# zakuro-ai/asr

Hardware: AMD Instinct MI355X
Metric: utterances/sec (10 s, 161-bin) DS2 5x1024 BiGRU CTC train step (higher is better)
Workload: dtype bf16

## Files before the change

asr_amd/_lib.py:

```python
from __future__ import annotations

import ctypes as C
import os
from typing import Optional

_HERE = os.path.dirname(os.path.abspath(__file__))
LIB_PATH = os.environ.get("DS2_LIB_PATH") or os.path.join(_HERE, "lib", "libds2hip.so")

_lib: Optional[C.CDLL] = None

vp, i32, i64, f32, f64, sz = C.c_void_p, C.c_int, C.c_longlong, C.c_float, C.c_double, C.c_size_t

SIGNATURES = {
    "ds2_version": (C.c_char_p, []),
    "ds2_last_error": (C.c_char_p, []),
    "ds2_device_info": (i32, [C.POINTER(i32), C.POINTER(i32), C.c_char_p, i32]),
    "ds2_debug_flags": (i32, [vp, i32]),
    "ds2_rnn_ctx_init": (i32, [vp, vp, vp, vp]),
    "ds2_memset_async": (i32, [vp, i32, sz, vp]),
    "ds2_ablation_build": (i32, []),
    "ds2_rnn_persistent_status": (i32, [vp, vp]),
    "ds2_rnn_persistent_counters": (i32, [vp, vp]),
    "ds2_rnn_poison_if_starved": (i32, [vp, vp, sz, vp]),
    "ds2_rnn_poison_seen": (i32, [vp]),
# ... 55 lines not shown
    "ds2_conv_wgrad_workspace_bytes": (sz, [i32, i32, i32]),
    "ds2_conv1_wgrad_f32": (i32, [vp, vp, vp, vp, i32, i32, i32, i32, vp, sz, vp]),
    "ds2_conv2_wgrad_f32": (i32, [vp, vp, vp, vp, i32, i32, i32, i32, vp, sz, vp]),
    "ds2_conv2_bf16_packed_bytes": (sz, [i32]),
    "ds2_conv2_pack_bf16": (i32, [vp, vp, vp, vp, vp]),
    "ds2_nhwc_bf16_f32": (i32, [vp, vp, i32, i32, i32, vp]),
    "ds2_conv2_fwd_bf16": (i32, [vp, vp, vp, vp, vp, i32, i32, i32, vp]),
    "ds2_conv2_dgrad_bf16": (i32, [vp, vp, vp, vp, i32, i32, i32, vp]),
    "ds2_conv_padded_pitch": (i32, [i32]),
    "ds2_padcast_bf16": (i32, [vp, vp, i64, i32, vp]),
    "ds2_conv2_wgrad_bf16_workspace_bytes": (sz, [i32, i32]),
    "ds2_conv2_wgrad_bf16": (i32, [vp, vp, vp, vp, i32, i32, i32, vp, sz, vp]),
    "ds2_conv2_wgrad_nhwc_bf16": (i32, [vp, vp, vp, vp, i32, i32, i32, vp, sz, vp]),
    "ds2_rnn_packed_bytes": (sz, [i32, i32, i32, i32]),
    "ds2_rnn_pack_whh": (i32, [i32, vp, vp, vp, i32, i32, vp]),
    "ds2_rnn_fwd_workspace_bytes": (sz, [i32, i32, i32]),
    "ds2_rnn_fwd_ex": (i32, [vp, i32, vp, vp, vp, vp, vp, vp, i32, i32, i32, i32, vp, vp, vp, sz, vp]),
    "ds2_rnn_fwd": (i32, [vp, i32, vp, vp, vp, vp, vp, vp, i32, i32, i32, i32, vp, vp, sz, vp]),
    "ds2_rnn_bwd_workspace_bytes": (sz, [i32, i32, i32, i32]),
    "ds2_rnn_bwd_ex": (i32, [vp, i32, vp, i32, vp, vp, vp, vp, vp, i32, i32, i32, i32, vp, vp, vp, vp, vp, sz, vp]),
    "ds2_rnn_bwd_bn": (i32, [vp, i32, vp, i32, vp, i32, vp, vp, vp, vp, vp, f32, vp, vp, vp, vp, vp, vp, i32, i32, i32, i32, vp, vp, vp, vp, vp, sz, vp]),
    "ds2_rnn_bwd_bn_xbf16": (i32, [vp, i32, vp, i32, vp, i32, vp, vp, vp, vp, vp, f32, vp, vp, vp, vp, vp, vp, i32, i32, i32, i32, vp, vp, vp, vp, vp, sz, vp]),
    "ds2_rnn_bias_grads": (i32, [i32, vp, i32, i32, vp, vp, vp]),
    "ds2_rnn_bwd": (i32, [vp, i32, vp, i32, vp, vp, vp, vp, vp, i32, i32, i32, i32, vp, vp, vp, sz, vp]),
    "ds2_ctc_workspace_bytes": (sz, [i32, i32, i32]),
    "ds2_ctc_loss_f32": (i32, [vp, i32, i32, i32, i32, vp, vp, vp, vp, i32, vp, vp, i32, f32, vp, sz, vp]),
    "ds2_ctc_batch_mean_f32": (i32, [vp, i32, vp, vp]),
    "ds2_add_i64": (i32, [vp, i32, i64, vp]),
    "ds2_softmax_rows_f32": (i32, [vp, i32, vp, i32, i32, i32, vp]),
    "ds2_greedy_decode_workspace_bytes": (sz, [i32, i32]),
    "ds2_greedy_decode_f32": (i32, [vp, i64, i64, i32, i32, i32, vp, i32, vp, vp, vp, vp, sz, vp]),
    "ds2_ctc_beam_max_width": (i32, []),
    "ds2_ctc_beam_workspace_bytes": (sz, [i32, i32, i32]),
    "ds2_ctc_beam_decode_f32": (i32, [vp, i64, i64, i32, i32, i32, vp, i32, i32, i32, f32, vp, vp, vp, vp, vp, sz, vp]),
    "ds2_ctc_beam_lm_max_candidates": (i32, []),
    "ds2_ctc_lm_packed_bytes": (sz, [i32, i32, i32, i32, i32]),
    "ds2_ctc_lm_pack": (i32, [i32, i32, vp, vp, vp, vp, i32, vp, vp, vp, i32, vp, i32, vp, i32, i32, vp, sz]),
    "ds2_ctc_lm_score": (i32, [vp, vp, i32, i32, C.POINTER(f32)]),
    "ds2_ctc_beam_decode_lm_f32": (i32, [vp, i64, i64, i32, i32, i32, vp, i32, i32, i32, f32, vp, sz, i32, i32, i32, f32, f32, vp, vp, vp, vp,
                                         vp, sz, vp]),
    "ds2_edit_distance_workspace_bytes": (sz, [i32, i64]),
# ... 16 lines not shown
    "ds2_tempo_workspace_bytes": (sz, [i32]),
    "ds2_tempo_gain_f32": (i32, [vp, i64, vp, vp, vp, i32, i32, f64, f64, f64, vp, i64, vp, vp, i32, vp, sz, vp]),
    "ds2_wave_unpack_f32": (i32, [vp, i64, i32, vp, vp, vp, i32, i32, vp, i64, vp]),
    "ds2_adamw_f32": (i32, [vp, vp, vp, vp, i64, f32, f32, f32, f32, f32, i32, f32, vp]),
    "ds2_adamw_gated_f32": (i32, [vp, vp, vp, vp, i64, f32, f32, f32, f32, f32, i32, f32, vp, vp]),
    "ds2_scale_f32": (i32, [vp, i64, f32, vp]),
    "ds2_bf16_residual_f32": (i32, [vp, vp, i64, vp]),
    "ds2_sum3_f32": (i32, [vp, vp, vp, vp, i64, vp]),
}


class TnProblem(C.Structure):
    _fields_ = [("A", vp), ("B", vp), ("C", vp), ("M", i32), ("N", i32), ("K", i32), ("lda", i32), ("ldb", i32), ("ldc", i32)]


class DS2LibraryError(RuntimeError):
    pass


def load() -> C.CDLL:
    global _lib
    if _lib is not None:
        return _lib
    if not os.path.exists(LIB_PATH):
        raise DS2LibraryError(
            f"{LIB_PATH} not found: build the HIP extension first "
            "(python -c 'import __graft_entry__ as g; g.build()'  or  make -C asr_amd/csrc). "
            "asr_amd has no CPU fallback.")
    lib = C.CDLL(LIB_PATH)
    for name, (res, args) in SIGNATURES.items():
# ... 22 lines not shown
```

asr_amd/csrc/ctc.hip:

```cpp
#include "common.h"
#include <math.h>

namespace {

constexpr float NEG_INF = -INFINITY;

__device__ __forceinline__ float fast_exp_(float x) { return __builtin_amdgcn_exp2f(x * 1.44269504088896340736f); }
__device__ __forceinline__ float fast_log_(float x) { return __builtin_amdgcn_logf(x) * 0.69314718055994530942f; }
__device__ __forceinline__ float lse2(float a, float b) {
  const float m = fmaxf(a, b);
  if (m == NEG_INF) return NEG_INF;
  return m + fast_log_(fast_exp_(a - m) + fast_exp_(b - m));
}
__device__ __forceinline__ float lse3(float a, float b, float c) {
  const float m = fmaxf(a, fmaxf(b, c));
  if (m == NEG_INF) return NEG_INF;
  return m + fast_log_(fast_exp_(a - m) + fast_exp_(b - m) + fast_exp_(c - m));
}

__global__ __launch_bounds__(256) void ctc_lse_kernel(const float* __restrict__ logits, int ld, int T, int Bn, int C,
                                                      const int* __restrict__ in_lens, float* __restrict__ lse) {
  const int row = blockIdx.x * 4 + (threadIdx.x >> 6);
  if (row >= T * Bn) return;
  const int t = row / Bn, b = row % Bn;
// ... 102 lines not shown
        }
        const float m = lse3(a0, a1, a2);
        const float v = (m == NEG_INF) ? NEG_INF : m + lp;
        cur[s] = v;
        out[(long long)t * Smax + s] = v;
      }
      __syncthreads();
      float* tmp = prev; prev = cur; cur = tmp;
    }
  }
  if (dirn == 0 && threadIdx.x == 0) {
    const float l1 = prev[S - 1];
    const float l2 = (S >= 2) ? prev[S - 2] : NEG_INF;
    nll[b] = -lse2(l1, l2);
  }
}

constexpr int TCH = 8;
__global__ __launch_bounds__(128) void ctc_grad_kernel(const float* __restrict__ logits, int ld, float* __restrict__ grad, int ldg, int T,
                                                       int Bn, int C, const int* __restrict__ targets,
                                                       const int* __restrict__ tgt_off, const int* __restrict__ in_lens,
                                                       const int* __restrict__ tgt_lens, const float* __restrict__ lse,
                                                       const float* __restrict__ ab, int Smax, const float* __restrict__ nll,
                                                       float scale) {
  extern __shared__ __attribute__((aligned(16))) float smem[];
  __shared__ float bred[2];
  const int b = blockIdx.y;
  const int t0 = blockIdx.x * TCH;
  const int Tb = min(in_lens[b], T), U = tgt_lens[b];
  const int S = 2 * U + 1;
// ... 96 lines not shown
}
}

extern "C" int ds2_ctc_batch_mean_f32(const float* nll_dev, int B, float* out_dev, void* stream) {
  DS2_REQUIRE(nll_dev && out_dev && B > 0, "ds2_ctc_batch_mean_f32: bad args");
  hipLaunchKernelGGL(batch_mean_kernel, dim3(1), dim3(64), 0, (hipStream_t)stream, nll_dev, B, out_dev);
  DS2_LAUNCH_CHECK("batch_mean_kernel");
  return 0;
}

extern "C" size_t ds2_ctc_workspace_bytes(int T, int B, int max_target_len) {
  const size_t Smax = 2 * (size_t)max_target_len + 1;
  return align_up((size_t)T * B * sizeof(float), 256) + 2 * (size_t)B * T * Smax * sizeof(float);
}

extern "C" int ds2_ctc_loss_f32(const float* logits, int ld, int T, int B, int C, const int* targets_dev, const int* tgt_off_dev,
                                const int* in_lens_dev, const int* tgt_lens_dev, int max_target_len, float* nll_dev,
                                float* grad, int ldg, float grad_scale, void* ws, size_t ws_bytes, void* stream) {
  DS2_REQUIRE(logits && targets_dev && tgt_off_dev && in_lens_dev && tgt_lens_dev && nll_dev, "ds2_ctc_loss_f32: null pointer");
  DS2_REQUIRE(T > 0 && B > 0 && C > 0 && max_target_len >= 0, "ds2_ctc_loss_f32: bad dims");
  DS2_REQUIRE(ws && ws_bytes >= ds2_ctc_workspace_bytes(T, B, max_target_len), "ds2_ctc_loss_f32: workspace too small");
  hipStream_t s = (hipStream_t)stream;
  const int Smax = 2 * max_target_len + 1;
  float* lse = (float*)ws;
  float* ab = (float*)((char*)ws + align_up((size_t)T * B * sizeof(float), 256));
  hipLaunchKernelGGL(ctc_lse_kernel, dim3(ceil_div(T * B, 4)), dim3(256), 0, s, logits, ld, T, B, C, in_lens_dev, lse);
  DS2_LAUNCH_CHECK("ctc_lse_kernel");
  int threads = ceil_div(Smax, 64) * 64;
  if (threads > 1024) threads = 1024;
  const size_t lds = (size_t)2 * Smax * sizeof(float);
  DS2_REQUIRE(lds <= 64 * 1024, "ds2_ctc_loss_f32: target too long for LDS lattice rows (Smax=%d)", Smax);
  hipLaunchKernelGGL(ctc_lattice_kernel, dim3(B, 2), dim3(threads), lds, s, logits, ld, T, B, C, targets_dev, tgt_off_dev,
                     in_lens_dev, tgt_lens_dev, (const float*)lse, ab, Smax, nll_dev);
  DS2_LAUNCH_CHECK("ctc_lattice_kernel");
  if (grad) {
    const size_t lds2 = ((size_t)C + Smax) * sizeof(float) + 3 * ((size_t)Smax / 2 + 1) * sizeof(int);
    DS2_REQUIRE(lds2 <= 64 * 1024, "ds2_ctc_loss_f32: C/S too large for LDS (C=%d Smax=%d)", C, Smax);
    hipLaunchKernelGGL(ctc_grad_kernel, dim3(ceil_div(T, TCH), B), dim3(128), lds2, s, logits, ld, grad, ldg, T, B, C, targets_dev,
                       tgt_off_dev, in_lens_dev, tgt_lens_dev, (const float*)lse, (const float*)ab, Smax, (const float*)nll_dev,
                       grad_scale);
    DS2_LAUNCH_CHECK("ctc_grad_kernel");
  }
  return 0;
}
```

asr_amd/csrc/optim.hip:

```cpp
#include "common.h"
#include <math.h>

namespace {

__global__ __launch_bounds__(256) void adamw_kernel(float* __restrict__ p, const float* __restrict__ g, float* __restrict__ m,
                                                    float* __restrict__ v, long long n, float lr, float b1, float b2, float eps,
                                                    float wd, float bc1, float bc2_sqrt, float gscale, const int* __restrict__ apply) {
  if (apply && *apply <= 0) return;
  const long long n4 = n / 4;
  const long long stride = (long long)gridDim.x * blockDim.x;
  for (long long i = (long long)blockIdx.x * blockDim.x + threadIdx.x; i < n4; i += stride) {
    f32x4 pp = reinterpret_cast<f32x4*>(p)[i];
    f32x4 gg = reinterpret_cast<const f32x4*>(g)[i] * gscale;
    f32x4 mm = reinterpret_cast<f32x4*>(m)[i];
    f32x4 vv = reinterpret_cast<f32x4*>(v)[i];
    pp *= (1.f - lr * wd);
    mm = b1 * mm + (1.f - b1) * gg;
    vv = b2 * vv + (1.f - b2) * gg * gg;
    f32x4 den;
    den.x = sqrtf(vv.x) / bc2_sqrt + eps; den.y = sqrtf(vv.y) / bc2_sqrt + eps;
    den.z = sqrtf(vv.z) / bc2_sqrt + eps; den.w = sqrtf(vv.w) / bc2_sqrt + eps;
    pp -= (lr / bc1) * mm / den;
    reinterpret_cast<f32x4*>(p)[i] = pp;
    reinterpret_cast<f32x4*>(m)[i] = mm;
// ... 101 lines not shown
  blocks = blocks < 1 ? 1 : (blocks > 8192 ? 8192 : blocks);
  hipLaunchKernelGGL(bf16_residual_kernel, dim3((unsigned)blocks), dim3(256), 0, (hipStream_t)stream, x, r, n / 4, n);
  DS2_LAUNCH_CHECK("bf16_residual_kernel");
  return 0;
}

extern "C" int ds2_sum3_f32(const float* a, const float* b, const float* c, float* out, long long n, void* stream) {
  DS2_REQUIRE(a && b && out && n >= 0 && (((uintptr_t)a | (uintptr_t)b | (uintptr_t)c | (uintptr_t)out) % 16) == 0, "ds2_sum3_f32: bad args");
  if (n == 0) return 0;
  long long blocks = (n / 4 + 255) / 256;
  blocks = blocks < 1 ? 1 : (blocks > 8192 ? 8192 : blocks);
  hipLaunchKernelGGL(sum3_kernel, dim3((unsigned)blocks), dim3(256), 0, (hipStream_t)stream, a, b, c, out, n / 4, n);
  DS2_LAUNCH_CHECK("sum3_kernel");
  return 0;
}
```

asr_amd/engine.py:

```python
from __future__ import annotations

from dataclasses import dataclass, field
from typing import Dict, List, Optional

import torch

from . import _lib, ops

Tensor = torch.Tensor
import os as _os
def _tune(name: str, default: str) -> str:
    return _os.environ.get(name, default) if _os.environ.get("DS2_EXPERIMENTAL") == "1" else default


OVERLAP_MODE = _tune("DS2_OVERLAP", "2")
OVERLAP_WGRAD = OVERLAP_MODE == "1"
WGRAD_TN = _tune("DS2_WGRAD_TN", "1") != "0"
CONV_STATS = _tune("DS2_CONV_STATS", "1") != "0"
FUSE_BN_BWD = _tune("DS2_FUSE_BN_BWD", "1") != "0"
WGRAD_SIDE = _tune("DS2_WGRAD_SIDE", "sk")
WGRAD_IDLE = _tune("DS2_WGRAD_IDLE", "1") != "0"
WGRAD_IDLE_MIN_CUS = int(_tune("DS2_WGRAD_IDLE_MIN_CUS", "64"))
F32_GEMM = _os.environ.get("DS2_F32_GEMM", "split")

# ... 188 lines not shown
    elif training:
        m2, v2 = ops.bn2d_stats(y2, *run(cp + "4"))
    else:
        m2, v2 = W[cp + "4.running_mean"], W[cp + "4.running_var"]
    xn0 = None
    if cfg.precision == "bf16":
        xin, xn0 = ops.bn2d_act_collapse(y2, lens_dev, m2, v2, W[cp + "4.weight"], W[cp + "4.bias"], want_f32=debug_acts, pad_to=64)
    else:
        a2 = ops.bn2d_act_fwd(y2, lens_dev, m2, v2, W[cp + "4.weight"], W[cp + "4.bias"])
        xin = ops.transpose_bft(a2, B, 32 * D2, T, to_tbf=True).view(M, 32 * D2)
        del a2
    if save:
        ctx.y1, ctx.a1, ctx.a1p, ctx.y2, ctx.st1, ctx.st2 = y1, a1, a1p, y2, (m1, v1), (m2, v2)

    mean = var = delta = None
    for l in range(L):
        lc = LayerCtx()
        bf = cfg.precision == "bf16"
        rmode = 1 if bf else (2 if (F32_RNN == "split" and H % 32 == 0) else 0)
        ws_f = ops.rnn_ws("fwd", G, B, H, rmode, x.device) if WS_PREARM else None
        folded = l > 0 and xin.dtype == torch.bfloat16
        if folded:
            bp = f"rnns.{l}.batch_norm.module."
            xn = xin
            w_bf, bias_eff, colscale, colshift = ops.wih_fold(W[f"rnns.{l}.wih_cat"], W[f"rnns.{l}.bih_cat"], var, W[bp + "weight"], W[bp + "bias"], delta,
                                                              ld=xn.shape[1])
            lc.wihT = ops.cast_transpose_bf16(W[f"rnns.{l}.wih_cat"])
            lc.mean, lc.var, lc.fold = delta, var, (colscale, colshift)
            gx = ops.gemm_bf16_nt(xn, w_bf, bias=bias_eff)
            del w_bf
        elif l > 0:
            bp = f"rnns.{l}.batch_norm.module."
            if not training:
                mean, var = W[bp + "running_mean"], W[bp + "running_var"]
            xn = (ops.bn1d_apply_bf16 if cfg.precision == "bf16" else ops.bn1d_apply)(xin, mean, var, W[bp + "weight"], W[bp + "bias"])
            lc.mean, lc.var = mean, var
        else:
            xn = xn0 if cfg.precision == "bf16" else xin
        if folded:
            pass
        elif cfg.precision == "bf16":
            if save:
                w_bf, lc.wihT = ops.cast_bf16_both(W[f"rnns.{l}.wih_cat"], ld_r=xn.shape[1])
            else:
                w_bf = ops.cast_bf16(W[f"rnns.{l}.wih_cat"], ld=xn.shape[1])
            gx = None
            if GX_BF16 and save and B % 8 == 0:
                gx = ops.gemm_bf16_nt_obf16(xn, w_bf, bias=W[f"rnns.{l}.bih_cat"])
            if gx is None:
                gx = ops.gemm_bf16_nt(xn, w_bf, bias=W[f"rnns.{l}.bih_cat"])
            del w_bf
        elif _f32_split_ok(M, 2 * G * H, xn.shape[1], H):
            lc.xs = ops.split_bf16(xn, 0, pad_rows=64 if save else 0)
            gx = ops.gemm_bf16_nt(lc.xs[:M], ops.split_bf16(W[f"rnns.{l}.wih_cat"], 1), bias=W[f"rnns.{l}.bih_cat"])
            if save:
                xn = None
        else:
            gx = ops.gemm(xn, W[f"rnns.{l}.wih_cat"], transB=True, bias=W[f"rnns.{l}.bih_cat"])
        wpf, wpb = ops.rnn_pack(G, W[f"rnns.{l}.whh_cat"], bf16=rmode)
        pack = bf and save and B % 8 == 0
        if pack:
            h_bf = (torch.empty(M, 2 * H, dtype=torch.bfloat16, device=x.device)
                    if (WGRAD_TN and OVERLAP_MODE == "2" and T > 1 and _BWD_PERSISTENT.get((ops.rnn_ctx_key(x.device), G, H, B), True)) else None)
            hsum = (torch.empty(2, (B + 15) // 16, H, dtype=torch.float32, device=x.device)
                    if (BN_FOLD and training and l + 1 < L and H % 8 == 0 and OVERLAP_MODE == "2" and T > 1
                        and (BN_FOLD_IDLE or not _wgrad_idle_schedule(x.device, B, H))) else None)
            hbuf, aux, rec = ops.rnn_fwd(G, gx, wpf, W[f"rnns.{l}.bhh_cat"], lens_dev, T, B, H, bf16=True, packed_gates=True, h_bf16=h_bf, ws=ws_f, hsum=hsum)
            if hsum is not None and not (ops.rnn_last_path(x.device) & 1):
                hsum = None
            gx = None
            lc.rec, lc.gshape = rec, (M, 2 * G * H)
            if h_bf is not None and (ops.rnn_last_path(x.device) & 1):
                lc.h_bf = h_bf
        else:
# ... 468 lines not shown
```

asr_amd/ops.py:

```python
from __future__ import annotations

import ctypes as C
import threading
from typing import Optional, Tuple

import torch

from . import _lib

Tensor = torch.Tensor
BN_EPS = 1e-5
BN_MOMENTUM = 0.1


def _ptr(t: Optional[Tensor]):
    return None if t is None else t.data_ptr()


def _stream():
    return torch.cuda.current_stream().cuda_stream


def _chk_f32(*ts):
    for t in ts:
# ... 835 lines not shown
    _lib.check(lib.ds2_conv2_wgrad_nhwc_bf16(a1n.data_ptr(), dy2n.data_ptr(), lens_dev.data_ptr(), dW2.data_ptr(), B, D1, T, ws.data_ptr(), wsb,
                                             _stream()), "ds2_conv2_wgrad_nhwc_bf16")


def rnn_pack(gates: int, whh: Tensor, bf16=False):
    _chk_f32(whh)
    assert whh.is_contiguous() and whh.dim() == 3
    lib = _lib.load()
    H = whh.size(2)
    wpf = torch.empty(lib.ds2_rnn_packed_bytes(gates, H, 0, int(bf16)), dtype=torch.uint8, device=whh.device)
    wpb = torch.empty(lib.ds2_rnn_packed_bytes(gates, H, 1, int(bf16)), dtype=torch.uint8, device=whh.device)
    _lib.check(lib.ds2_rnn_pack_whh(gates, whh.data_ptr(), wpf.data_ptr(), wpb.data_ptr(), H, int(bf16), _stream()), "ds2_rnn_pack_whh")
    return wpf, wpb


def rnn_ws(kind: str, gates: int, B: int, H: int, bf16, device) -> Tensor:
    lib = _lib.load()
    n = lib.ds2_rnn_fwd_workspace_bytes(B, H, int(bf16)) if kind == "fwd" else lib.ds2_rnn_bwd_workspace_bytes(gates, B, H, int(bf16))
    ws = _ws(n, device)
    _lib.check(lib.ds2_memset_async(ws.data_ptr(), 0xff, ws.numel(), _stream()), "ds2_memset_async")
    return ws


def _take_ws(ws: Optional[Tensor], need: int, device):
    if ws is None:
        return _ws(need, device), False
    assert ws.numel() >= need and ws.device == torch.device(device)
    return ws, True


# ... 146 lines not shown
                                  _ptr(dhn_bf16), _ptr(bias_part), ws.data_ptr(), wsb, _stream()))
    rc = call(None)
    if rc == 1:
        rc = call(torch.empty(T * B, H, dtype=torch.float32, device=dyn.device))
    _lib.check(rc, "ds2_rnn_bwd_bn")


def rnn_bias_grads(gates: int, bias_part: Tensor, dbih: Tensor, dbhh: Tensor):
    _chk_f32(bias_part, dbih, dbhh)
    B, _, _, H = bias_part.shape
    assert bias_part.is_contiguous() and dbih.is_contiguous() and dbhh.is_contiguous() and dbih.numel() == 2 * gates * H == dbhh.numel()
    _lib.check(_lib.load().ds2_rnn_bias_grads(gates, bias_part.data_ptr(), B, H, dbih.data_ptr(), dbhh.data_ptr(), _stream()), "ds2_rnn_bias_grads")


def ctc_loss(logits: Tensor, targets_dev: Tensor, tgt_off_dev: Tensor, in_lens_dev: Tensor, tgt_lens_dev: Tensor, max_tgt: int,
             grad_scale: float, want_grad: bool = True):
    _chk_f32(logits)
    lib = _lib.load()
    T, B, Cc = logits.shape
    assert logits.stride(2) == 1 and logits.stride(0) == B * logits.stride(1)
    ld = logits.stride(1)
    nll = torch.empty(B, dtype=torch.float32, device=logits.device)
    grad = torch.empty(T, B, Cc, dtype=torch.float32, device=logits.device) if want_grad else None
    wsb = lib.ds2_ctc_workspace_bytes(T, B, max_tgt)
    ws = _ws(wsb, logits.device)
    _lib.check(lib.ds2_ctc_loss_f32(logits.data_ptr(), ld, T, B, Cc, targets_dev.data_ptr(), tgt_off_dev.data_ptr(),
                                    in_lens_dev.data_ptr(), tgt_lens_dev.data_ptr(), int(max_tgt), nll.data_ptr(), _ptr(grad), Cc,
                                    float(grad_scale), ws.data_ptr(), wsb, _stream()), "ds2_ctc_loss_f32")
    return nll, grad


def ctc_batch_mean(nll: Tensor) -> Tensor:
    _chk_f32(nll)
    assert nll.dim() == 1 and nll.is_contiguous()
    out = torch.empty(1, dtype=torch.float32, device=nll.device)
    _lib.check(_lib.load().ds2_ctc_batch_mean_f32(nll.data_ptr(), nll.numel(), out.data_ptr(), _stream()), "ds2_ctc_batch_mean_f32")
    return out


def add_i64(x: Tensor, v: int = 1):
    assert x.dtype == torch.int64 and x.is_contiguous() and x.is_cuda
    _lib.check(_lib.load().ds2_add_i64(x.data_ptr(), x.numel(), int(v), _stream()), "ds2_add_i64")

# ... 290 lines not shown
```

include/ds2hip.h:

```cpp
#ifndef DS2HIP_H
#define DS2HIP_H

#include <stddef.h>
#include <stdint.h>

#ifdef __cplusplus
extern "C" {
#endif

const char* ds2_version(void);
const char* ds2_last_error(void);
int ds2_device_info(int* cu_count, int* wave_size, char* arch, int arch_len);
int ds2_ablation_build(void);

typedef struct ds2_rnn_ctx {
  int size;
  int persist_fwd, persist_bwd;
  int cooldown;
  int rearm_calls;
  int starved_total;
  int last_path;
  int last_bwd_kind;
  int debug_flags;
  int ws_prearmed;
// ... 107 lines not shown
size_t ds2_chanstats_from_partials_workspace_bytes(void);
int ds2_chanstats_from_partials(const float* part, int nblk, int C, double count, float* mean, float* var, float* run_mean, float* run_var,
                                float momentum, void* ws, size_t ws_bytes, void* stream);
int ds2_conv2_dgrad_bf16(const void* dy2_nhwc, const void* wd0, const void* wd1, float* da1, int B, int D1, int T, void* stream);

int ds2_conv_padded_pitch(int T);
int ds2_padcast_bf16(const float* src, void* dst, long long R, int T, void* stream);
size_t ds2_conv2_wgrad_bf16_workspace_bytes(int B, int D1);
int ds2_conv2_wgrad_bf16(const void* a1p, const void* dy2p, const int* lens_dev, float* dW2, int B, int D1, int T, void* ws, size_t ws_bytes,
                         void* stream);
int ds2_conv2_wgrad_nhwc_bf16(const void* a1_nhwc, const void* dy2_nhwc, const int* lens_dev, float* dW2, int B, int D1, int T, void* ws,
                              size_t ws_bytes, void* stream);

size_t ds2_rnn_packed_bytes(int gates, int H, int which , int bf16);
int ds2_rnn_pack_whh(int gates, const float* whh, void* wp_fwd, void* wp_bwd, int H, int bf16, void* stream);
int ds2_rnn_persistent_status(ds2_rnn_ctx* ctx, int* out8);
int ds2_rnn_persistent_counters(const ds2_rnn_ctx* ctx, int* out2);
int ds2_rnn_poison_if_starved(ds2_rnn_ctx* ctx, float* buf, size_t n, void* stream);
int ds2_rnn_poison_seen(const ds2_rnn_ctx* ctx);
int ds2_rnn_step_gate(const ds2_rnn_ctx* ctx, const float* loss_dev, int* flag_dev, void* stream);
int ds2_rnn_persistent_enable(ds2_rnn_ctx* ctx, int forward, int backward);
int ds2_rnn_bwd_ksplit_footprint(int gates, int H, int* out3);
int ds2_rnn_last_path(const ds2_rnn_ctx* ctx);
size_t ds2_rnn_fwd_workspace_bytes(int B, int H, int bf16);
int ds2_rnn_fwd(ds2_rnn_ctx* ctx, int gates, float* gx, const void* wp_fwd, const float* bhh, float* hbuf, float* aux, const int* lens_dev, int T, int B,
                int H, int bf16, void* gates_bf16, void* ws, size_t ws_bytes, void* stream);
int ds2_rnn_fwd_ex(ds2_rnn_ctx* ctx, int gates, float* gx, const void* wp_fwd, const float* bhh, float* hbuf, float* aux, const int* lens_dev, int T, int B,
                   int H, int bf16, void* gates_bf16, void* h_bf16, void* ws, size_t ws_bytes, void* stream);
int ds2_rnn_fwd_x(ds2_rnn_ctx* ctx, int gates, float* gx, const void* gx_bf16, const void* wp_fwd, const float* bhh, float* hbuf, float* aux,
                  const int* lens_dev, int T, int B, int H, void* gates_bf16, void* h_bf16, float* hsum, void* ws, size_t ws_bytes, void* stream);
// ... 9 lines not shown
                   const float* bn_gamma, const float* bn_s0, const float* bn_s1, float bn_eps, float* dy_scratch, float* gx, float* aux,
                   const float* hbuf, const void* wp_bwd, const int* lens_dev, int T, int B, int H, int bf16, void* dgx_bf16,
                   const void* gates_bf16, void* dhn_bf16, float* bias_part, void* ws, size_t ws_bytes, void* stream);

int ds2_rnn_bwd_bn_xbf16(ds2_rnn_ctx* ctx, int gates, const float* dyn, int lddyn, const void* bn_x_bf16, int ldx, const float* bn_mean,
                         const float* bn_var, const float* bn_gamma, const float* bn_s0, const float* bn_s1, float bn_eps, float* dy_scratch, float* gx,
                         float* aux, const float* hbuf, const void* wp_bwd, const int* lens_dev, int T, int B, int H, int bf16, void* dgx_bf16,
                         const void* gates_bf16, void* dhn_bf16, float* bias_part, void* ws, size_t ws_bytes, void* stream);

int ds2_rnn_bias_grads(int gates, const float* bias_part, int B, int H, float* dbih, float* dbhh, void* stream);

size_t ds2_ctc_workspace_bytes(int T, int B, int max_target_len);
int ds2_ctc_loss_f32(const float* logits, int ld, int T, int B, int C, const int* targets_dev, const int* tgt_off_dev,
                     const int* in_lens_dev, const int* tgt_lens_dev, int max_target_len, float* nll_dev, float* grad, int ldg,
                     float grad_scale, void* ws, size_t ws_bytes, void* stream);

int ds2_ctc_batch_mean_f32(const float* nll_dev, int B, float* out_dev, void* stream);

int ds2_softmax_rows_f32(const float* x, int ldx, float* y, int ldy, int rows, int C, void* stream);

size_t ds2_greedy_decode_workspace_bytes(int B, int T);
int ds2_greedy_decode_f32(const float* probs, long long ld_b, long long ld_t, int B, int T, int C, const int* sizes_dev, int blank,
                          int* ids, int* offs, int* out_len, void* ws, size_t ws_bytes, void* stream);

int ds2_ctc_beam_max_width(void);
size_t ds2_ctc_beam_workspace_bytes(int B, int T, int beam_width);
int ds2_ctc_beam_decode_f32(const float* probs, long long ld_b, long long ld_t, int B, int T, int C, const int* sizes_dev, int blank,
                            int beam_width, int cutoff_top_n, float cutoff_prob, int* labels, int* offsets, int* lens, float* scores,
                            void* ws, size_t ws_bytes, void* stream);

// ... 63 lines not shown
```

Measured before the change: 2786.

## Batch per-layer bf16 weight prep into one kernel and add wave-level CTC lattice

Adds a single table-driven weight_prep kernel that packs W_hh for the recurrent kernels and casts/transposes W_ih to bf16 for every layer in one launch, replacing several per-layer cast and pack launches in the forward pass. It also adds a single-wavefront CTC alpha/beta lattice kernel that uses DPP lane shifts and register-prefetched logits instead of LDS and block barriers, used by default when the padded label length fits in 128. The trade-off is more complex code, extra live bf16 weight buffers allocated up front, and a fast path that only covers short targets.

```diff
diff --git a/asr_amd/_lib.py b/asr_amd/_lib.py
--- a/asr_amd/_lib.py
+++ b/asr_amd/_lib.py
@@ -93,6 +93,7 @@
     "ds2_conv2_wgrad_nhwc_bf16": (i32, [vp, vp, vp, vp, i32, i32, i32, vp, sz, vp]),
     "ds2_rnn_packed_bytes": (sz, [i32, i32, i32, i32]),
     "ds2_rnn_pack_whh": (i32, [i32, vp, vp, vp, i32, i32, vp]),
+    "ds2_weight_prep_bf16": (i32, [vp, i32, vp]),
     "ds2_rnn_fwd_workspace_bytes": (sz, [i32, i32, i32]),
     "ds2_rnn_fwd_ex": (i32, [vp, i32, vp, vp, vp, vp, vp, vp, i32, i32, i32, i32, vp, vp, vp, sz, vp]),
     "ds2_rnn_fwd": (i32, [vp, i32, vp, vp, vp, vp, vp, vp, i32, i32, i32, i32, vp, vp, sz, vp]),
@@ -104,6 +105,7 @@
     "ds2_rnn_bwd": (i32, [vp, i32, vp, i32, vp, vp, vp, vp, vp, i32, i32, i32, i32, vp, vp, vp, sz, vp]),
     "ds2_ctc_workspace_bytes": (sz, [i32, i32, i32]),
     "ds2_ctc_loss_f32": (i32, [vp, i32, i32, i32, i32, vp, vp, vp, vp, i32, vp, vp, i32, f32, vp, sz, vp]),
+    "ds2_ctc_loss_ex_f32": (i32, [vp, i32, i32, i32, i32, vp, vp, vp, vp, i32, vp, vp, i32, f32, i32, vp, sz, vp]),
     "ds2_ctc_batch_mean_f32": (i32, [vp, i32, vp, vp]),
     "ds2_add_i64": (i32, [vp, i32, i64, vp]),
     "ds2_softmax_rows_f32": (i32, [vp, i32, vp, i32, i32, i32, vp]),
@@ -150,6 +152,11 @@
     _fields_ = [("A", vp), ("B", vp), ("C", vp), ("M", i32), ("N", i32), ("K", i32), ("lda", i32), ("ldb", i32), ("ldc", i32)]
 
 
+class PrepLayer(C.Structure):
+    _fields_ = [("whh", vp), ("wp_fwd", vp), ("wp_bwd", vp), ("wih", vp), ("wih_t", vp), ("wih_r", vp),
+                ("gates", i32), ("H", i32), ("R", i32), ("Cc", i32), ("ld_wih", i32), ("ld_t", i32), ("ld_r", i32), ("reserved", i32)]
+
+
 class DS2LibraryError(RuntimeError):
     pass
 
diff --git a/asr_amd/csrc/ctc.hip b/asr_amd/csrc/ctc.hip
--- a/asr_amd/csrc/ctc.hip
+++ b/asr_amd/csrc/ctc.hip
@@ -140,6 +140,122 @@
     const float l2 = (S >= 2) ? prev[S - 2] : NEG_INF;
     nll[b] = -lse2(l1, l2);
   }
+}
+
+constexpr int WPF = 8;
+typedef float f32x2_a4 __attribute__((ext_vector_type(2), aligned(4)));
+template <int CTRL>
+__device__ __forceinline__ float wave_shift1(float v) {
+  return __int_as_float(__builtin_amdgcn_update_dpp(__float_as_int(NEG_INF), __float_as_int(v), CTRL, 0xf, 0xf, false));
+}
+__device__ __forceinline__ float lse3_sel(float a, float b, float c) {
+  const float m = fmaxf(a, fmaxf(b, c));
+  const float r = m + fast_log_(fast_exp_(a - m) + fast_exp_(b - m) + fast_exp_(c - m));
+  return (m == NEG_INF) ? NEG_INF : r;
+}
+__device__ __forceinline__ float lse2_sel(float a, float b) {
+  const float m = fmaxf(a, fmaxf(b, NEG_INF));
+  const float r = m + fast_log_(fast_exp_(a - m) + fast_exp_(b - m));
+  return (m == NEG_INF) ? NEG_INF : r;
+}
+
+template <int DIRN>
+__device__ __forceinline__ void ctc_lattice_wave_body(const float* __restrict__ logits, int ld, int T, int Bn, const int* __restrict__ lab,
+                                                      int b, int Tb, int U, const float* __restrict__ lse, float* __restrict__ out, int Smax,
+                                                      float* __restrict__ nll) {
+  const int S = 2 * U + 1;
+  const int l = threadIdx.x;
+  const bool actE = 2 * l < S, actO = 2 * l + 1 < S;
+  const int step = DIRN == 0 ? 1 : -1;
+  const int tfirst = DIRN == 0 ? 0 : Tb - 1;
+  int cls = 0;
+  bool skip = false;
+  if (actO) {
+    cls = lab[l];
+    if (DIRN == 0) skip = (l >= 1) && (cls != lab[l - 1]);
+    else skip = (l + 1 < U) && (cls != lab[l + 1]);
+  }
+  const long long lg_stride = (long long)step * Bn * ld;
+  const int ls_stride = step * Bn, out_stride = step * Smax;
+  int vz;
+  asm volatile("v_mov_b32 %0, 0" : "=v"(vz));
+  const float* lgb = logits + ((long long)tfirst * Bn + b) * ld + vz;
+  const float* lsp = lse + (long long)tfirst * Bn + b + vz;
+  float* op = out + (long long)tfirst * Smax + (actE ? 2 * l : 0);
+  const int last = Tb - 1;
+  auto fetch = [&](int i, float& lgE, float& lgO, float& ls) {
+    const int ii = i < last ? i : last;
+    ls = lsp[(long long)ii * ls_stride];
+    lgE = lgb[(long long)ii * lg_stride];
+    lgO = lgb[(long long)ii * lg_stride + cls];
+  };
+  float E = NEG_INF, O = NEG_INF;
+  auto store_pair = [&]() {
+    if (actO) *reinterpret_cast<f32x2_a4*>(op) = f32x2_a4{E, O};
+    else if (actE) op[0] = E;
+  };
+  {
+    float lgE, lgO, ls;
+    fetch(0, lgE, lgO, ls);
+    const float eE = lgE - ls, eO = lgO - ls;
+    if (DIRN == 0) { if (l == 0) { E = eE; if (actO) O = eO; } }
+    else { if (2 * l == S - 1) E = eE; if (actO && 2 * l + 1 == S - 2) O = eO; }
+    store_pair();
+  }
+  auto frame = [&](float lgE, float lgO, float ls) {
+    const float lpE = actE ? lgE - ls : NEG_INF, lpO = actO ? lgO - ls : NEG_INF;
+    op += out_stride;
+    float mE, mO;
+    if (DIRN == 0) {
+      const float Om = wave_shift1<0x138>(O);
+      mE = lse2_sel(E, Om);
+      mO = lse3_sel(O, E, skip ? Om : NEG_INF);
+    } else {
+      const float Ep = wave_shift1<0x130>(E), Op = wave_shift1<0x130>(O);
+      mE = lse2_sel(E, O);
+      mO = lse3_sel(O, Ep, skip ? Op : NEG_INF);
+    }
+    E = (mE == NEG_INF) ? NEG_INF : mE + lpE;
+    O = (mO == NEG_INF) ? NEG_INF : mO + lpO;
+    store_pair();
+  };
+  float rE[WPF], rO[WPF], rL[WPF];
+#pragma unroll
+  for (int k = 0; k < WPF; ++k) fetch(1 + k, rE[k], rO[k], rL[k]);
+  int i0 = 1;
+  for (; i0 + WPF <= Tb; i0 += WPF) {
+#pragma unroll
+    for (int k = 0; k < WPF; ++k) {
+      const float lgE = rE[k], lgO = rO[k], ls = rL[k];
+      fetch(i0 + k + WPF, rE[k], rO[k], rL[k]);
+      frame(lgE, lgO, ls);
+    }
+  }
+#pragma unroll
+  for (int k = 0; k < WPF - 1; ++k)
+    if (i0 + k < Tb) frame(rE[k], rO[k], rL[k]);
+  if (DIRN == 0) {
+    const float l1 = __shfl(E, U, 64);
+    const float l2 = __shfl(O, U >= 1 ? U - 1 : 0, 64);
+    if (l == 0) nll[b] = -lse2(l1, (S >= 2) ? l2 : NEG_INF);
+  }
+}
+
+__global__ __launch_bounds__(64) void ctc_lattice_wave_kernel(const float* __restrict__ logits, int ld, int T, int Bn, int C,
+                                                              const int* __restrict__ targets, const int* __restrict__ tgt_off,
+                                                              const int* __restrict__ in_lens, const int* __restrict__ tgt_lens,
+                                                              const float* __restrict__ lse, float* __restrict__ ab, int Smax,
+                                                              float* __restrict__ nll) {
+  const int b = blockIdx.x, dirn = blockIdx.y;
+  const int Tb = min(in_lens[b], T), U = tgt_lens[b];
+  float* out = ab + (((long long)dirn * Bn + b) * T) * Smax;
+  if (Tb <= 0) {
+    if (dirn == 0 && threadIdx.x == 0) nll[b] = (U == 0) ? 0.f : INFINITY;
+    return;
+  }
+  const int* lab = targets + tgt_off[b];
+  if (dirn == 0) ctc_lattice_wave_body<0>(logits, ld, T, Bn, lab, b, Tb, U, lse, out, Smax, nll);
+  else ctc_lattice_wave_body<1>(logits, ld, T, Bn, lab, b, Tb, U, lse, out, Smax, nll);
 }
 
 constexpr int TCH = 8;
@@ -266,11 +382,12 @@
   return align_up((size_t)T * B * sizeof(float), 256) + 2 * (size_t)B * T * Smax * sizeof(float);
 }
 
-extern "C" int ds2_ctc_loss_f32(const float* logits, int ld, int T, int B, int C, const int* targets_dev, const int* tgt_off_dev,
-                                const int* in_lens_dev, const int* tgt_lens_dev, int max_target_len, float* nll_dev,
-                                float* grad, int ldg, float grad_scale, void* ws, size_t ws_bytes, void* stream) {
+extern "C" int ds2_ctc_loss_ex_f32(const float* logits, int ld, int T, int B, int C, const int* targets_dev, const int* tgt_off_dev,
+                                   const int* in_lens_dev, const int* tgt_lens_dev, int max_target_len, float* nll_dev, float* grad, int ldg,
+                                   float grad_scale, int lattice, void* ws, size_t ws_bytes, void* stream) {
   DS2_REQUIRE(logits && targets_dev && tgt_off_dev && in_lens_dev && tgt_lens_dev && nll_dev, "ds2_ctc_loss_f32: null pointer");
   DS2_REQUIRE(T > 0 && B > 0 && C > 0 && max_target_len >= 0, "ds2_ctc_loss_f32: bad dims");
+  DS2_REQUIRE(lattice == 0 || lattice == 1, "ds2_ctc_loss_ex_f32: lattice must be 0 or 1");
   DS2_REQUIRE(ws && ws_bytes >= ds2_ctc_workspace_bytes(T, B, max_target_len), "ds2_ctc_loss_f32: workspace too small");
   hipStream_t s = (hipStream_t)stream;
   const int Smax = 2 * max_target_len + 1;
@@ -278,13 +395,19 @@
   float* ab = (float*)((char*)ws + align_up((size_t)T * B * sizeof(float), 256));
   hipLaunchKernelGGL(ctc_lse_kernel, dim3(ceil_div(T * B, 4)), dim3(256), 0, s, logits, ld, T, B, C, in_lens_dev, lse);
   DS2_LAUNCH_CHECK("ctc_lse_kernel");
-  int threads = ceil_div(Smax, 64) * 64;
-  if (threads > 1024) threads = 1024;
-  const size_t lds = (size_t)2 * Smax * sizeof(float);
-  DS2_REQUIRE(lds <= 64 * 1024, "ds2_ctc_loss_f32: target too long for LDS lattice rows (Smax=%d)", Smax);
-  hipLaunchKernelGGL(ctc_lattice_kernel, dim3(B, 2), dim3(threads), lds, s, logits, ld, T, B, C, targets_dev, tgt_off_dev,
-                     in_lens_dev, tgt_lens_dev, (const float*)lse, ab, Smax, nll_dev);
-  DS2_LAUNCH_CHECK("ctc_lattice_kernel");
+  if (lattice == 0 && Smax <= 128) {
+    hipLaunchKernelGGL(ctc_lattice_wave_kernel, dim3(B, 2), dim3(64), 0, s, logits, ld, T, B, C, targets_dev, tgt_off_dev, in_lens_dev,
+                       tgt_lens_dev, (const float*)lse, ab, Smax, nll_dev);
+    DS2_LAUNCH_CHECK("ctc_lattice_wave_kernel");
+  } else {
+    int threads = ceil_div(Smax, 64) * 64;
+    if (threads > 1024) threads = 1024;
+    const size_t lds = (size_t)2 * Smax * sizeof(float);
+    DS2_REQUIRE(lds <= 64 * 1024, "ds2_ctc_loss_f32: target too long for LDS lattice rows (Smax=%d)", Smax);
+    hipLaunchKernelGGL(ctc_lattice_kernel, dim3(B, 2), dim3(threads), lds, s, logits, ld, T, B, C, targets_dev, tgt_off_dev,
+                       in_lens_dev, tgt_lens_dev, (const float*)lse, ab, Smax, nll_dev);
+    DS2_LAUNCH_CHECK("ctc_lattice_kernel");
+  }
   if (grad) {
     const size_t lds2 = ((size_t)C + Smax) * sizeof(float) + 3 * ((size_t)Smax / 2 + 1) * sizeof(int);
     DS2_REQUIRE(lds2 <= 64 * 1024, "ds2_ctc_loss_f32: C/S too large for LDS (C=%d Smax=%d)", C, Smax);
@@ -295,3 +418,10 @@
   }
   return 0;
 }
+
+extern "C" int ds2_ctc_loss_f32(const float* logits, int ld, int T, int B, int C, const int* targets_dev, const int* tgt_off_dev,
+                                const int* in_lens_dev, const int* tgt_lens_dev, int max_target_len, float* nll_dev,
+                                float* grad, int ldg, float grad_scale, void* ws, size_t ws_bytes, void* stream) {
+  return ds2_ctc_loss_ex_f32(logits, ld, T, B, C, targets_dev, tgt_off_dev, in_lens_dev, tgt_lens_dev, max_target_len, nll_dev, grad, ldg,
+                             grad_scale, 0, ws, ws_bytes, stream);
+}
diff --git a/asr_amd/csrc/optim.hip b/asr_amd/csrc/optim.hip
--- a/asr_amd/csrc/optim.hip
+++ b/asr_amd/csrc/optim.hip
@@ -139,3 +139,212 @@
   DS2_LAUNCH_CHECK("sum3_kernel");
   return 0;
 }
+
+namespace {
+
+typedef __bf16 pbf16x8 __attribute__((ext_vector_type(8)));
+typedef __bf16 pbf16x4 __attribute__((ext_vector_type(4)));
+
+enum { PREP_PACK_TILE = 0, PREP_PACK_VEC = 1, PREP_CAST_T = 2 };
+constexpr int PREP_MAX_JOBS = 32;
+struct PrepJob {
+  const float* src;
+  void* d0;
+  void* d1;
+  int kind, first;
+  int G, H;
+  int R, Cc, lds, ldt, ldr, vec, gx;
+};
+struct PrepTable {
+  int njobs;
+  PrepJob job[PREP_MAX_JOBS];
+};
+
+constexpr int PT = 68;
+
+__device__ __forceinline__ pbf16x8 to_bf16x8(const float* v) {
+  pbf16x8 o;
+#pragma unroll
+  for (int e = 0; e < 8; ++e) o[e] = (__bf16)v[e];
+  return o;
+}
+
+__device__ __forceinline__ void prep_pack_tile(const PrepJob& jb, int lb, float* tile) {
+  const int G = jb.G, H = jb.H, GH = G * H;
+  const int rt = (GH + 63) >> 6, ct = (H + 63) >> 6;
+  const int dir = lb / (rt * ct), rem = lb % (rt * ct);
+  const int r0 = (rem / ct) * 64, c0 = (rem % ct) * 64;
+  const int nsl = H >> 4, nch = (H + 31) >> 5, nchb = (GH + 31) >> 5;
+  const float* src = jb.src + (long long)dir * GH * H;
+  const int tid = threadIdx.x;
+#pragma unroll
+  for (int pass = 0; pass < 4; ++pass) {
+    const int rl = pass * 16 + (tid >> 4), cl = (tid & 15) * 4;
+    const int r = r0 + rl, c = c0 + cl;
+    f32x4 q = {0.f, 0.f, 0.f, 0.f};
+    if (r < GH && c < H) q = *reinterpret_cast<const f32x4*>(src + (long long)r * H + c);
+    *reinterpret_cast<f32x4*>(tile + rl * PT + cl) = q;
+  }
+  __syncthreads();
+#pragma unroll
+  for (int p = 0; p < 2; ++p) {
+    const int v = p * 256 + tid, lane = v & 63, cc = (v >> 6) & 1, i = v >> 7;
+    const int row = r0 + 16 * i, c = (c0 >> 5) + cc;
+    if (row < GH && c < nch) {
+      const int g = row / H, slice = (row % H) >> 4;
+      const float* t = tile + (16 * i + (lane & 15)) * PT + cc * 32 + (lane >> 4) * 8;
+      float x[8];
+      *reinterpret_cast<f32x4*>(x) = *reinterpret_cast<const f32x4*>(t);
+      *reinterpret_cast<f32x4*>(x + 4) = *reinterpret_cast<const f32x4*>(t + 4);
+      reinterpret_cast<pbf16x8*>(jb.d0)[((((long long)dir * nsl + slice) * G + g) * nch + c) * 64 + lane] = to_bf16x8(x);
+    }
+  }
+#pragma unroll
+  for (int p = 0; p < 2; ++p) {
+    const int v = p * 256 + tid, lane = v & 63, sj = (v >> 6) & 3, ci = v >> 8;
+    const int cb = (r0 >> 5) + ci, slice = (c0 >> 4) + sj;
+    if (cb < nchb && slice < nsl) {
+      const float* t = tile + (ci * 32 + (lane >> 4) * 8) * PT + sj * 16 + (lane & 15);
+      float x[8];
+#pragma unroll
+      for (int e = 0; e < 8; ++e) x[e] = t[e * PT];
+      reinterpret_cast<pbf16x8*>(jb.d1)[(((long long)dir * nsl + slice) * nchb + cb) * 64 + lane] = to_bf16x8(x);
+    }
+  }
+}
+
+__device__ __forceinline__ void prep_pack_vec(const PrepJob& jb, int lb) {
+  const int G = jb.G, H = jb.H;
+  const int nsl = (H + 15) >> 4, nch = (H + 31) >> 5, nchb = (G * H + 31) >> 5;
+  const long long nf = (long long)2 * nsl * G * nch * 64, nb = (long long)2 * nsl * nchb * 64;
+  const long long i = (long long)lb * 256 + threadIdx.x;
+  if (i >= nf + nb) return;
+  const bool fwd = i < nf;
+  const long long ii = fwd ? i : i - nf;
+  const int lane = (int)(ii & 63);
+  long long r = ii >> 6;
+  float v[8];
+  if (fwd) {
+    const int c = r % nch; r /= nch;
+    const int g = r % G; r /= G;
+    const int slice = r % nsl, dir = r / nsl;
+    const int j = slice * 16 + (lane & 15), k0 = c * 32 + (lane >> 4) * 8;
+    const float* src = jb.src + ((long long)dir * G * H + g * H + j) * H + k0;
+#pragma unroll
+    for (int e = 0; e < 8; ++e) v[e] = (j < H && k0 + e < H) ? src[e] : 0.f;
+  } else {
+    const int c = r % nchb; r /= nchb;
+    const int slice = r % nsl, dir = r / nsl;
+    const int j = slice * 16 + (lane & 15), k0 = c * 32 + (lane >> 4) * 8;
+    const float* src = jb.src + ((long long)dir * G * H + k0) * H + j;
+#pragma unroll
+    for (int e = 0; e < 8; ++e) v[e] = (j < H && k0 + e < G * H) ? src[(long long)e * H] : 0.f;
+  }
+  reinterpret_cast<pbf16x8*>(fwd ? jb.d0 : jb.d1)[ii] = to_bf16x8(v);
+}
+
+__device__ __forceinline__ void prep_cast_t(const PrepJob& jb, int lb, float* tile) {
+  const int R = jb.R, Cc = jb.Cc, ldt = jb.ldt, ldr = jb.ldr;
+  __bf16* dstT = (__bf16*)jb.d0;
+  __bf16* dstR = (__bf16*)jb.d1;
+  const int r0 = (lb / jb.gx) * 64, c0 = (lb % jb.gx) * 64;
+  const int tid = threadIdx.x;
+#pragma unroll
+  for (int pass = 0; pass < 4; ++pass) {
+    const int rl = pass * 16 + (tid >> 4), cl = (tid & 15) * 4;
+    const int r = r0 + rl, c = c0 + cl;
+    float v[4] = {0.f, 0.f, 0.f, 0.f};
+    if (r < R) {
+      const float* sp = jb.src + (long long)r * jb.lds + c;
+      if (jb.vec && c + 4 <= Cc) {
+        const f32x4 q = *reinterpret_cast<const f32x4*>(sp);
+        v[0] = q.x; v[1] = q.y; v[2] = q.z; v[3] = q.w;
+      } else {
+#pragma unroll
+        for (int j = 0; j < 4; ++j) v[j] = (c + j < Cc) ? sp[j] : 0.f;
+      }
+      if (dstR && c < ldr) *reinterpret_cast<pbf16x4*>(dstR + (long long)r * ldr + c) = pbf16x4{(__bf16)v[0], (__bf16)v[1], (__bf16)v[2], (__bf16)v[3]};
+    }
+#pragma unroll
+    for (int j = 0; j < 4; ++j) tile[rl * 65 + cl + j] = v[j];
+  }
+  __syncthreads();
+#pragma unroll
+  for (int pass = 0; pass < 2; ++pass) {
+    const int cl = pass * 32 + (tid >> 3), rl = (tid & 7) * 8;
+    const int c = c0 + cl, r = r0 + rl;
+    if (c < Cc && r < ldt) {
+      float x[8];
+#pragma unroll
+      for (int j = 0; j < 8; ++j) x[j] = tile[(rl + j) * 65 + cl];
+      *reinterpret_cast<pbf16x8*>(dstT + (long long)c * ldt + r) = to_bf16x8(x);
+    }
+  }
+}
+
+__global__ __launch_bounds__(256) void weight_prep_kernel(const PrepTable tab) {
+  __shared__ __attribute__((aligned(16))) float tile[64 * PT];
+  const int bid = blockIdx.x;
+  int j = 0;
+  while (j + 1 < tab.njobs && bid >= tab.job[j + 1].first) ++j;
+  const PrepJob& jb = tab.job[j];
+  const int lb = bid - jb.first;
+  if (jb.kind == PREP_PACK_TILE) prep_pack_tile(jb, lb, tile);
+  else if (jb.kind == PREP_PACK_VEC) prep_pack_vec(jb, lb);
+  else prep_cast_t(jb, lb, tile);
+}
+
+}
+
+extern "C" int ds2_weight_prep_bf16(const ds2_prep_layer* layers, int n, void* stream) {
+  DS2_REQUIRE(layers && n > 0, "ds2_weight_prep_bf16: bad args");
+  PrepTable tab;
+  tab.njobs = 0;
+  long long blocks = 0;
+  auto flush = [&]() -> int {
+    if (tab.njobs == 0) return 0;
+    hipLaunchKernelGGL(weight_prep_kernel, dim3((unsigned)blocks), dim3(256), 0, (hipStream_t)stream, tab);
+    DS2_LAUNCH_CHECK("weight_prep_kernel");
+    tab.njobs = 0;
+    blocks = 0;
+    return 0;
+  };
+  for (int i = 0; i < n; ++i) {
+    const ds2_prep_layer& L = layers[i];
+    if (tab.njobs + 2 > PREP_MAX_JOBS && flush()) return 1;
+    if (L.whh) {
+      DS2_REQUIRE(L.gates == 1 || L.gates == 3 || L.gates == 4, "ds2_weight_prep_bf16: gates must be 1, 3 or 4");
+      DS2_REQUIRE(L.wp_fwd && L.wp_bwd && L.H > 0 && (L.H % 4) == 0 && ((uintptr_t)L.whh % 16) == 0 && ((uintptr_t)L.wp_fwd % 16) == 0 &&
+                      ((uintptr_t)L.wp_bwd % 16) == 0,
+                  "ds2_weight_prep_bf16: bad W_hh arguments (layer %d)", i);
+      PrepJob& jb = tab.job[tab.njobs++];
+      jb = PrepJob{};
+      jb.src = L.whh; jb.d0 = L.wp_fwd; jb.d1 = L.wp_bwd; jb.G = L.gates; jb.H = L.H; jb.first = (int)blocks;
+      if ((L.H % 16) == 0) {
+        jb.kind = PREP_PACK_TILE;
+        blocks += 2LL * ceil_div(L.gates * L.H, 64) * ceil_div(L.H, 64);
+      } else {
+        jb.kind = PREP_PACK_VEC;
+        const long long nsl = ceil_div(L.H, 16);
+        const long long nv = 2 * nsl * L.gates * ceil_div(L.H, 32) * 64 + 2 * nsl * ceil_div(L.gates * L.H, 32) * 64;
+        blocks += (nv + 255) / 256;
+      }
+    }
+    if (L.wih) {
+      DS2_REQUIRE(L.wih_t && L.R > 0 && L.Cc > 0 && L.ld_wih >= L.Cc && L.ld_t >= L.R && (L.ld_t % 8) == 0 && ((uintptr_t)L.wih_t % 16) == 0,
+                  "ds2_weight_prep_bf16: bad W_ih arguments (layer %d)", i);
+      DS2_REQUIRE(!L.wih_r || (L.ld_r >= L.Cc && L.ld_r <= ceil_div(L.Cc, 64) * 64 && (L.ld_r % 8) == 0 && ((uintptr_t)L.wih_r % 16) == 0),
+                  "ds2_weight_prep_bf16: bad row-major pitch (layer %d, ld_r=%d)", i, L.ld_r);
+      PrepJob& jb = tab.job[tab.njobs++];
+      jb = PrepJob{};
+      jb.kind = PREP_CAST_T;
+      jb.src = L.wih; jb.d0 = L.wih_t; jb.d1 = L.wih_r; jb.first = (int)blocks;
+      jb.R = L.R; jb.Cc = L.Cc; jb.lds = L.ld_wih; jb.ldt = L.ld_t; jb.ldr = L.wih_r ? L.ld_r : 0;
+      jb.vec = ((L.ld_wih % 4) == 0) && (((uintptr_t)L.wih % 16) == 0);
+      jb.gx = ceil_div(L.wih_r ? (L.Cc > L.ld_r ? L.Cc : L.ld_r) : L.Cc, 64);
+      blocks += (long long)jb.gx * ceil_div(L.ld_t, 64);
+    }
+    DS2_REQUIRE(blocks < (1LL << 31), "ds2_weight_prep_bf16: too many tiles");
+  }
+  return flush();
+}
diff --git a/asr_amd/engine.py b/asr_amd/engine.py
--- a/asr_amd/engine.py
+++ b/asr_amd/engine.py
@@ -226,9 +226,15 @@
         ctx.y1, ctx.a1, ctx.a1p, ctx.y2, ctx.st1, ctx.st2 = y1, a1, a1p, y2, (m1, v1), (m2, v2)
 
     mean = var = delta = None
+    bf = cfg.precision == "bf16"
+    prep = None
+    if bf and save:
+        may_fold = (BN_FOLD and training and B % 8 == 0 and H % 8 == 0 and OVERLAP_MODE == "2" and T > 1
+                    and (BN_FOLD_IDLE or not _wgrad_idle_schedule(x.device, B, H)))
+        prep = ops.weight_prep_bf16([(G, W[f"rnns.{l}.whh_cat"], W[f"rnns.{l}.wih_cat"],
+                                      xn0.shape[1] if l == 0 else (None if may_fold else ops._pad8(H))) for l in range(L)])
     for l in range(L):
         lc = LayerCtx()
-        bf = cfg.precision == "bf16"
         rmode = 1 if bf else (2 if (F32_RNN == "split" and H % 32 == 0) else 0)
         ws_f = ops.rnn_ws("fwd", G, B, H, rmode, x.device) if WS_PREARM else None
         folded = l > 0 and xin.dtype == torch.bfloat16
@@ -237,7 +243,7 @@
             xn = xin
             w_bf, bias_eff, colscale, colshift = ops.wih_fold(W[f"rnns.{l}.wih_cat"], W[f"rnns.{l}.bih_cat"], var, W[bp + "weight"], W[bp + "bias"], delta,
                                                               ld=xn.shape[1])
-            lc.wihT = ops.cast_transpose_bf16(W[f"rnns.{l}.wih_cat"])
+            lc.wihT = prep[l][2] if prep is not None else ops.cast_transpose_bf16(W[f"rnns.{l}.wih_cat"])
             lc.mean, lc.var, lc.fold = delta, var, (colscale, colshift)
             gx = ops.gemm_bf16_nt(xn, w_bf, bias=bias_eff)
             del w_bf
@@ -253,7 +259,10 @@
             pass
         elif cfg.precision == "bf16":
             if save:
-                w_bf, lc.wihT = ops.cast_bf16_both(W[f"rnns.{l}.wih_cat"], ld_r=xn.shape[1])
+                if prep is not None and prep[l][3] is not None and prep[l][3].shape[1] == xn.shape[1]:
+                    lc.wihT, w_bf = prep[l][2], prep[l][3]
+                else:
+                    w_bf, lc.wihT = ops.cast_bf16_both(W[f"rnns.{l}.wih_cat"], ld_r=xn.shape[1])
             else:
                 w_bf = ops.cast_bf16(W[f"rnns.{l}.wih_cat"], ld=xn.shape[1])
             gx = None
@@ -269,7 +278,9 @@
                 xn = None
         else:
             gx = ops.gemm(xn, W[f"rnns.{l}.wih_cat"], transB=True, bias=W[f"rnns.{l}.bih_cat"])
-        wpf, wpb = ops.rnn_pack(G, W[f"rnns.{l}.whh_cat"], bf16=rmode)
+        wpf, wpb = prep[l][:2] if prep is not None else ops.rnn_pack(G, W[f"rnns.{l}.whh_cat"], bf16=rmode)
+        if prep is not None:
+            prep[l] = None
         pack = bf and save and B % 8 == 0
         if pack:
             h_bf = (torch.empty(M, 2 * H, dtype=torch.bfloat16, device=x.device)
diff --git a/asr_amd/ops.py b/asr_amd/ops.py
--- a/asr_amd/ops.py
+++ b/asr_amd/ops.py
@@ -873,6 +873,33 @@
     return wpf, wpb
 
 
+def weight_prep_bf16(layers):
+    lib = _lib.load()
+    tab = (_lib.PrepLayer * len(layers))()
+    out = []
+    for e, (gates, whh, wih, ld_r) in zip(tab, layers):
+        wpf = wpb = wt = wr = None
+        if whh is not None:
+            _chk_f32(whh)
+            assert whh.is_contiguous() and whh.dim() == 3
+            dev, H = whh.device, whh.size(2)
+            wpf = torch.empty(lib.ds2_rnn_packed_bytes(gates, H, 0, 1), dtype=torch.uint8, device=dev)
+            wpb = torch.empty(lib.ds2_rnn_packed_bytes(gates, H, 1, 1), dtype=torch.uint8, device=dev)
+            e.whh, e.wp_fwd, e.wp_bwd, e.gates, e.H = whh.data_ptr(), wpf.data_ptr(), wpb.data_ptr(), gates, H
+        if wih is not None:
+            _chk_f32(wih)
+            R, Cc = wih.shape
+            wt = torch.empty(Cc, _pad8(R), dtype=torch.bfloat16, device=wih.device)
+            e.wih, e.wih_t, e.R, e.Cc, e.ld_wih, e.ld_t = wih.data_ptr(), wt.data_ptr(), R, Cc, _row_pitch(wih), wt.size(1)
+            if ld_r is not None:
+                assert ld_r >= Cc and ld_r % 8 == 0
+                wr = torch.empty(R, ld_r, dtype=torch.bfloat16, device=wih.device)
+                e.wih_r, e.ld_r = wr.data_ptr(), ld_r
+        out.append((wpf, wpb, wt, wr))
+    _lib.check(lib.ds2_weight_prep_bf16(tab, len(layers), _stream()), "ds2_weight_prep_bf16")
+    return out
+
+
 def rnn_ws(kind: str, gates: int, B: int, H: int, bf16, device) -> Tensor:
     lib = _lib.load()
     n = lib.ds2_rnn_fwd_workspace_bytes(B, H, int(bf16)) if kind == "fwd" else lib.ds2_rnn_bwd_workspace_bytes(gates, B, H, int(bf16))
@@ -1049,7 +1076,7 @@
 
 
 def ctc_loss(logits: Tensor, targets_dev: Tensor, tgt_off_dev: Tensor, in_lens_dev: Tensor, tgt_lens_dev: Tensor, max_tgt: int,
-             grad_scale: float, want_grad: bool = True):
+             grad_scale: float, want_grad: bool = True, lattice: int = 0, return_ab: bool = False):
     _chk_f32(logits)
     lib = _lib.load()
     T, B, Cc = logits.shape
@@ -1059,9 +1086,15 @@
     grad = torch.empty(T, B, Cc, dtype=torch.float32, device=logits.device) if want_grad else None
     wsb = lib.ds2_ctc_workspace_bytes(T, B, max_tgt)
     ws = _ws(wsb, logits.device)
-    _lib.check(lib.ds2_ctc_loss_f32(logits.data_ptr(), ld, T, B, Cc, targets_dev.data_ptr(), tgt_off_dev.data_ptr(),
-                                    in_lens_dev.data_ptr(), tgt_lens_dev.data_ptr(), int(max_tgt), nll.data_ptr(), _ptr(grad), Cc,
-                                    float(grad_scale), ws.data_ptr(), wsb, _stream()), "ds2_ctc_loss_f32")
+    if return_ab:
+        ws.zero_()
+    _lib.check(lib.ds2_ctc_loss_ex_f32(logits.data_ptr(), ld, T, B, Cc, targets_dev.data_ptr(), tgt_off_dev.data_ptr(),
+                                       in_lens_dev.data_ptr(), tgt_lens_dev.data_ptr(), int(max_tgt), nll.data_ptr(), _ptr(grad), Cc,
+                                       float(grad_scale), int(lattice), ws.data_ptr(), wsb, _stream()), "ds2_ctc_loss_ex_f32")
+    if return_ab:
+        Smax = 2 * int(max_tgt) + 1
+        off = (T * B * 4 + 255) // 256 * 256
+        return nll, grad, ws[off:off + 2 * B * T * Smax * 4].view(torch.float32).view(2, B, T, Smax).clone()
     return nll, grad
 
 
diff --git a/include/ds2hip.h b/include/ds2hip.h
--- a/include/ds2hip.h
+++ b/include/ds2hip.h
@@ -145,6 +145,12 @@
 
 size_t ds2_rnn_packed_bytes(int gates, int H, int which , int bf16);
 int ds2_rnn_pack_whh(int gates, const float* whh, void* wp_fwd, void* wp_bwd, int H, int bf16, void* stream);
+typedef struct ds2_prep_layer {
+  const float* whh; void* wp_fwd; void* wp_bwd;
+  const float* wih; void* wih_t; void* wih_r;
+  int gates, H, R, Cc, ld_wih, ld_t, ld_r, reserved;
+} ds2_prep_layer;
+int ds2_weight_prep_bf16(const ds2_prep_layer* layers, int n, void* stream);
 int ds2_rnn_persistent_status(ds2_rnn_ctx* ctx, int* out8);
 int ds2_rnn_persistent_counters(const ds2_rnn_ctx* ctx, int* out2);
 int ds2_rnn_poison_if_starved(ds2_rnn_ctx* ctx, float* buf, size_t n, void* stream);
@@ -184,6 +190,9 @@
 int ds2_ctc_loss_f32(const float* logits, int ld, int T, int B, int C, const int* targets_dev, const int* tgt_off_dev,
                      const int* in_lens_dev, const int* tgt_lens_dev, int max_target_len, float* nll_dev, float* grad, int ldg,
                      float grad_scale, void* ws, size_t ws_bytes, void* stream);
+int ds2_ctc_loss_ex_f32(const float* logits, int ld, int T, int B, int C, const int* targets_dev, const int* tgt_off_dev,
+                        const int* in_lens_dev, const int* tgt_lens_dev, int max_target_len, float* nll_dev, float* grad, int ldg,
+                        float grad_scale, int lattice, void* ws, size_t ws_bytes, void* stream);
 
 int ds2_ctc_batch_mean_f32(const float* nll_dev, int B, float* out_dev, void* stream);
 
```

Result: faster. 2815, median of 6 (+1.1%).
